# BrooksLabUCSC/splicedice

Measured on AMD Instinct MI355X. Metric: PS-matrix entries/sec (junctions x samples), higher is better.
Workload: dtype int32 counts -> f32 PS; 1 GPU; quant 2000000 junctions x 500 samples per GPU (north_star target size), cluster+PS; junctions_per_gpu=2000000, samples=500, counts=one seeded block of 200000 rows repeated down the matrix, parallelism=junction shards x1, one rank per GPU

## Files before the change

splicedice_amd/csrc/cluster_fast.hip:

```cpp
#include "common.h"

#ifndef SDICE_CLUSTER_ABLATE
#define SDICE_CLUSTER_ABLATE 0
#endif
#define SD_ABL(a, bit) (SDICE_CLUSTER_ABLATE && ((a).ablate & (bit)))

int sd_cluster_legacy(sdice_ctx* ctx, int64_t n, const int32_t* d_chrom, const int32_t* d_left, const int32_t* d_right,
                      const int8_t* d_strand, int32_t* d_row_of, int64_t* d_row_ptr, int64_t* nnz_out);

namespace {

constexpr int SPB = 8;
constexpr int BUCKET_MEAN = 2048;
constexpr int MAX_BUCKETS = 4096;
constexpr int SLOT_FACTOR = 8;
constexpr int64_t FAST_MAX_N = (int64_t)MAX_BUCKETS * BUCKET_MEAN;

enum : unsigned long long { ST_INVALID = 1, ST_SLOT_OVERFLOW = 2, ST_DUP = 4, ST_COL_OVERFLOW = 8, ST_LOOKBACK = 16 };
constexpr int SB_FLAGS = 0, SB_NNZ = 2, SB_MAXLEN = 32, SB_REACH = 64, SB_WORDS = 96;
constexpr int SB_STICKY = SB_WORDS, SB_ALLOC_WORDS = SB_WORDS + 8;
constexpr int SB_SLOTS = 32;

struct FastArgs {
    const int32_t* chrom; const int32_t* left; const int32_t* right; const int8_t* strand;
// ... 274 lines not shown
                for (int k = 0; k < K; ++k) {
                    const int kp = k ^ j;
                    if (kp > k) {
                        bool up;
                        if (k2 < K) up = (k & k2) == 0;
                        else if (k2 >= 64 * K) up = true;
                        else up = (lane & (k2 / K)) == 0;
                        const bool sw = up ? key[kp] < key[k] : key[kp] > key[k];
                        const uint64_t tk = key[k];
                        key[k] = sw ? key[kp] : tk;
                        key[kp] = sw ? tk : key[kp];
                    }
                }
            }
        }
    }
}

constexpr int SS_NB = 16;
constexpr int SS_MIN = 512, SS_MAX = 6400, SS_SUB_CAP = 1024;
constexpr int SS_KPT = (SS_MAX + SORT_T_ - 1) / SORT_T_;
static_assert((8192 - SS_MAX) * 8 >= SS_MAX * 2 && (8192 - SS_MAX) * 8 >= 256 * 12, "scratch behind the keys must hold the lists / the sample");

template <int K>
__device__ __forceinline__ void ss_sort_sub(const uint64_t* kb, const unsigned short* list, int n, int lane, uint64_t (&key)[16]) {
    uint64_t k_[K];
#pragma unroll
    for (int k = 0; k < K; ++k) {
        const int p = k * 64 + lane;
        k_[k] = p < n ? kb[list[p]] : ~0ull;
    }
    wave_sort_u64<K>(k_, lane);
#pragma unroll
    for (int k = 0; k < K; ++k) key[k] = k_[k];
}

__device__ __forceinline__ bool lds_sample_sort(uint64_t* kb, int count, int t) {
    __shared__ unsigned s_cnt[SS_NB], s_base[SS_NB + 1], s_max;
    __shared__ uint64_t s_spl[SS_NB];
    const int lane = t & 63, w = __builtin_amdgcn_readfirstlane(t >> 6);
    uint64_t* smp = kb + count;
    const int ns = count <= 2048 ? 128 : 256;
    const int per = ns / SS_NB;
    unsigned* rnk = reinterpret_cast<unsigned*>(smp + ns);
    unsigned short* list = reinterpret_cast<unsigned short*>(kb + count);
    __syncthreads();
    if (t < ns) { smp[t] = kb[(int)((int64_t)t * count / ns)]; rnk[t] = 0u; }
    if (t < SS_NB) s_cnt[t] = 0u;
    __syncthreads();
    {
        const int i = t & (ns - 1), chunk = SORT_T_ / ns, c = t / ns, len = ns / chunk;
        const uint64_t me = smp[i];
        unsigned below = 0;
        for (int j = c * len; j < c * len + len; ++j) below += smp[j] < me ? 1u : 0u;
        atomicAdd(&rnk[i], below);
    }
    __syncthreads();
    if (t < ns) {
        const unsigned r = rnk[t];
        if (r > 0 && r % (unsigned)per == 0) s_spl[r / (unsigned)per - 1] = smp[t];
    }
    __syncthreads();
    int where[SS_KPT];
#pragma unroll
    for (int q = 0; q < SS_KPT; ++q) {
        const int i = q * SORT_T_ + t;
        const bool act = i < count;
        int b = 0;
        if (act) {
            const uint64_t key = kb[i];
            int lo = 0, hi = SS_NB - 1;
            while (lo < hi) {
                const int mid = (lo + hi) >> 1;
                const bool le = s_spl[mid] <= key;
                lo = le ? mid + 1 : lo;
                hi = le ? hi : mid;
            }
            b = lo;
        }
        unsigned long long m = __ballot(act);
#pragma unroll
        for (int bit = 0; bit < 4; ++bit) {
            const unsigned long long bb = __ballot((b >> bit) & 1);
            m &= ((b >> bit) & 1) ? bb : ~bb;
        }
        unsigned basew = 0;
        if (act) {
            const int leader = __ffsll((long long)m) - 1;
            if (lane == leader) basew = atomicAdd(&s_cnt[b], (unsigned)__popcll(m));
            basew = (unsigned)__shfl((int)basew, leader);
        }
        where[q] = act ? (int)(((basew + (unsigned)__popcll(m & ((1ull << lane) - 1ull))) << 4) | (unsigned)b) : -1;
    }
    __syncthreads();
    if (w == 0) {
        const unsigned c = lane < SS_NB ? s_cnt[lane] : 0u;
        unsigned x = c, mx = c;
#pragma unroll
        for (int o = 1; o < SS_NB; o <<= 1) {
            const unsigned y = (unsigned)__shfl_up((int)x, o);
            if (lane >= o) x += y;
        }
#pragma unroll
        for (int o = 8; o > 0; o >>= 1) mx = max(mx, (unsigned)__shfl_xor((int)mx, o));
        if (lane < SS_NB) s_base[lane + 1] = x;
        if (lane == 0) { s_base[0] = 0u; s_max = mx; }
    }
    __syncthreads();
    if (s_max > (unsigned)SS_SUB_CAP) return false;
#pragma unroll
    for (int q = 0; q < SS_KPT; ++q)
        if (where[q] >= 0) list[s_base[where[q] & 15] + (unsigned)(where[q] >> 4)] = (unsigned short)(q * SORT_T_ + t);
    __syncthreads();
    const int n = (int)s_cnt[w];
    const unsigned base = s_base[w];
    uint64_t key[16];
    const int K = n <= 128 ? 2 : n <= 256 ? 4 : n <= 512 ? 8 : 16;
    if (K == 2) ss_sort_sub<2>(kb, list + base, n, lane, key);
    else if (K == 4) ss_sort_sub<4>(kb, list + base, n, lane, key);
    else if (K == 8) ss_sort_sub<8>(kb, list + base, n, lane, key);
    else ss_sort_sub<16>(kb, list + base, n, lane, key);
    __syncthreads();
#pragma unroll
    for (int k = 0; k < 16; ++k) {
        const int p = lane * K + k;
        if (k < K && p < n) kb[base + p] = key[k];
    }
    __syncthreads();
    return true;
}

constexpr int SORT_T = SORT_T_;
constexpr int SORT_WAVES = SORT_T / 64;
constexpr int RDX_CAP = 8192;
constexpr int RDX_IDX_BITS = 13;
constexpr int SORT_LDS_ELEMS = 4096;
constexpr size_t SORT_LDS_BYTES = (size_t)RDX_CAP * 8;
static_assert(SORT_LDS_BYTES >= (size_t)SORT_LDS_ELEMS * 16, "unpacked fallback must fit");

__device__ __forceinline__ int bits_u32(uint32_t v) { return v ? 32 - __clz(v) : 0; }

__global__ void __launch_bounds__(SORT_T, 8) bucket_sort_kernel(FastArgs a) {
    extern __shared__ uint4 lds_elems[];
    __shared__ unsigned long long wsum[SORT_WAVES];
    __shared__ uint32_t red[5][SORT_WAVES];
    __shared__ uint32_t s_dup;
    const int t = threadIdx.x, b = blockIdx.x, lane = t & 63, w = __builtin_amdgcn_readfirstlane(t >> 6);
    if (a.sb[SB_FLAGS] & (ST_INVALID | ST_SLOT_OVERFLOW)) return;
    const int count = (int)a.cursor[b];
    unsigned long long part = 0;
    for (int i = t; i < b; i += SORT_T) part += a.cursor[i];
#pragma unroll
    for (int o = 32; o > 0; o >>= 1) part += __shfl_xor(part, o);
    if (lane == 0) wsum[w] = part;
    if (t == 0) s_dup = 0;
    __syncthreads();
    int64_t start = 0;
    for (int k = 0; k < SORT_WAVES; ++k) start += (int64_t)wsum[k];
    if (count == 0) return;
    uint4* src = a.slots + (int64_t)b * a.slot_cap;

    int total_bits = 99, bl = 0, bn = 0;
    uint32_t cmin = 0, lmin = 0;
    const bool small = count <= RDX_CAP && count <= a.lds_cap;
    if (small) {
        uint32_t c0 = 0xffffffffu, c1 = 0, l0 = 0xffffffffu, l1 = 0, n1 = 0;
        for (int i = t; i < count; i += SORT_T) {
            const uint4 e = src[i];
            c0 = min(c0, e.x); c1 = max(c1, e.x); l0 = min(l0, e.y); l1 = max(l1, e.y); n1 = max(n1, (e.z >> 1) - e.y);
        }
#pragma unroll
        for (int o = 32; o > 0; o >>= 1) {
            c0 = min(c0, (uint32_t)__shfl_xor((int)c0, o)); c1 = max(c1, (uint32_t)__shfl_xor((int)c1, o));
            l0 = min(l0, (uint32_t)__shfl_xor((int)l0, o)); l1 = max(l1, (uint32_t)__shfl_xor((int)l1, o));
            n1 = max(n1, (uint32_t)__shfl_xor((int)n1, o));
        }
        if (lane == 0) { red[0][w] = c0; red[1][w] = c1; red[2][w] = l0; red[3][w] = l1; red[4][w] = n1; }
        __syncthreads();
        for (int k = 0; k < SORT_WAVES; ++k) {
            c0 = min(c0, red[0][k]); c1 = max(c1, red[1][k]); l0 = min(l0, red[2][k]); l1 = max(l1, red[3][k]);
            n1 = max(n1, red[4][k]);
        }
        cmin = c0; lmin = l0;
        bl = bits_u32(l1 - l0); bn = bits_u32(n1);
        total_bits = bits_u32(c1 - c0) + bl + bn + 1;
    }
    uint32_t dup = 0;
    auto emit_all = [&](auto get) {
        for (int i0 = 0; i0 < count; i0 += SORT_T) {
            const int i = i0 + t;
            const bool act = i < count;
            uint32_t rr = 0, blk = 0xffffffffu;
            if (act) {
                const uint4 e = get(i);
                const int64_t r = start + i;
                a.rowC[r] = e.x; a.rowL[r] = e.y; a.rowR2[r] = e.z;
                a.row_of[e.w] = (int32_t)r;
                rr = e.z >> 1;
                blk = (uint32_t)(r >> 6);
            }
            const uint32_t blk0 = (uint32_t)__shfl((int)blk, 0);
            uint32_t m0 = (act && blk == blk0) ? rr : 0u, m1 = (act && blk != blk0) ? rr : 0u;
#pragma unroll
            for (int o = 32; o > 0; o >>= 1) {
                m0 = max(m0, (uint32_t)__shfl_xor((int)m0, o));
                m1 = max(m1, (uint32_t)__shfl_xor((int)m1, o));
            }
            if (lane == 0 && blk0 != 0xffffffffu) {
                if (m0) atomicMax(&a.bmax64[blk0], m0);
                if (m1) atomicMax(&a.bmax64[blk0 + 1], m1);
            }
        }
    };
    if (small && total_bits + RDX_IDX_BITS <= 64) {
        uint64_t* kb0 = reinterpret_cast<uint64_t*>(lds_elems);
        for (int i = t; i < count; i += SORT_T) {
            const uint4 e = src[i];
            uint64_t k = (((uint64_t)(e.x - cmin) << bl) | (uint64_t)(e.y - lmin)) << bn;
            k = ((k | (uint64_t)((e.z >> 1) - e.y)) << 1) | (uint64_t)(e.z & 1u);
            kb0[i] = (k << RDX_IDX_BITS) | (uint64_t)i;
        }
        int P = 1;
        while (P < count) P <<= 1;
        bool sorted_already = false;
        if (a.sample_sort && count >= SS_MIN && count <= SS_MAX && !SD_ABL(a, 1)) sorted_already = lds_sample_sort(kb0, count, t);
        if (sorted_already) {}
        else if (P > 1 && !SD_ABL(a, 1)) bitonic_sort_u64(kb0, count, P, t, SORT_T); else __syncthreads();
        const uint64_t* sorted = kb0;
        for (int i = t; i + 1 < count; i += SORT_T)
            if ((sorted[i] >> RDX_IDX_BITS) == (sorted[i + 1] >> RDX_IDX_BITS)) dup = 1;
        if (!SD_ABL(a, 2)) emit_all([&](int i) { return src[sorted[i] & ((1u << RDX_IDX_BITS) - 1u)]; });
    } else {
        int P = 1;
        while (P < count) P <<= 1;
        uint4* buf;
        if (count <= SORT_LDS_ELEMS && count <= a.lds_cap) {
            for (int i = t; i < count; i += SORT_T) lds_elems[i] = src[i];
            buf = lds_elems;
            if (P > 1) bitonic_sort<true, uint4>(buf, count, P, t, SORT_T); else __syncthreads();
        } else {
            buf = src;
            bitonic_sort<false, uint4>(buf, count, P, t, SORT_T);
        }
        for (int i = t; i + 1 < count; i += SORT_T) {
            const uint4 e = buf[i], f = buf[i + 1];
            if (f.x == e.x && f.y == e.y && f.z == e.z) dup = 1;
        }
        emit_all([&](int i) { return buf[i]; });
    }
    if (dup) s_dup = 1;
    __syncthreads();
    if (t == 0 && s_dup) { atomicOr(&a.sb[SB_FLAGS], (unsigned long long)ST_DUP); atomicOr(&a.sb[SB_STICKY], (unsigned long long)ST_DUP); }
}

constexpr unsigned long long LB_A = 1ull << 62, LB_P = 2ull << 62, LB_MASK = (1ull << 62) - 1;

__device__ __forceinline__ unsigned long long ld_agent(const unsigned long long* p) {
    return __hip_atomic_load(p, __ATOMIC_RELAXED, __HIP_MEMORY_SCOPE_AGENT);
}
__device__ __forceinline__ void st_agent(unsigned long long* p, unsigned long long v) {
    __hip_atomic_store(p, v, __ATOMIC_RELAXED, __HIP_MEMORY_SCOPE_AGENT);
}

__device__ __forceinline__ unsigned long long lookback_exclusive(unsigned long long* state, int tile, unsigned long long agg,
                                                                 int lane, unsigned long long* sb, bool fail) {
    if (lane == 0) st_agent(&state[tile], (tile == 0 ? LB_P : LB_A) | agg);
    unsigned long long excl = 0;
    int idx = tile - 1;
    unsigned spins = fail && tile == 1 ? (1u << 21) : 0u;
    while (idx >= 0) {
        const int j = idx - lane;
        const unsigned long long v = j >= 0 ? ld_agent(&state[j]) : LB_P;
        const unsigned flag = (unsigned)(v >> 62);
        const unsigned long long empty = __ballot(flag == 0u);
        const unsigned long long pm = __ballot(flag == 2u);
        const int first_p = pm ? __ffsll((long long)pm) - 1 : 64;
        const unsigned long long need = first_p >= 63 ? ~0ull : ((1ull << (first_p + 1)) - 1ull);
        if ((empty & need) || (fail && tile == 1)) {
            if (++spins > (1u << 21)) {
                if (lane == 0) { atomicOr(&sb[SB_FLAGS], (unsigned long long)ST_LOOKBACK); atomicOr(&sb[SB_STICKY], (unsigned long long)ST_LOOKBACK); }
                break;
            }
            __builtin_amdgcn_s_sleep(2);
            continue;
        }
        unsigned long long x = lane <= first_p ? (v & LB_MASK) : 0ull;
#pragma unroll
        for (int o = 32; o > 0; o >>= 1) x += __shfl_xor(x, o);
        excl += x;
        if (first_p < 64) break;
        idx -= 64;
    }
    if (lane == 0 && tile != 0) st_agent(&state[tile], LB_P | (excl + agg));
    return excl;
}

template <int T>
struct NbCfg {
    static constexpr int HB = 256;
    static constexpr int HF = 128;
    static constexpr int W = T + HB + HF;
    static constexpr int STAGE = 11 * T;
    static constexpr int KMAX = 16;
    static constexpr int WIN_WORDS = 6 * W;
    static constexpr int UNION_WORDS = WIN_WORDS > STAGE ? WIN_WORDS : STAGE;
};

template <class Emit>
__device__ __forceinline__ void walk_back_global(const FastArgs& a, int q, uint32_t c, uint32_t l, uint32_t st, uint32_t maxlen,
                                                 Emit emit) {
    while (q >= 0) {
        const uint32_t qc = a.rowC[q], ql = a.rowL[q], qr = a.rowR2[q];
        if (qc != c || ql + maxlen < l) break;
        if ((q & 63) == 63 && a.bmax64[q >> 6] < l) { q -= 64; continue; }
        if ((qr & 1u) == st && (qr >> 1) >= l) emit(q);
        --q;
    }
}
template <class Emit>
__device__ __forceinline__ void walk_fwd_global(const FastArgs& a, int q, int n, uint32_t c, uint32_t rgt, uint32_t st, Emit emit) {
    while (q < n) {
        const uint32_t qc = a.rowC[q], ql = a.rowL[q], qr = a.rowR2[q];
        if (qc != c || ql > rgt) break;
        if ((qr & 1u) == st) emit(q);
        ++q;
    }
}

template <int T>
__global__ void __launch_bounds__(T, 8) neighbours_kernel(FastArgs a) {
    typedef NbCfg<T> Cfg;
    constexpr int W = Cfg::W, KMAX = Cfg::KMAX;
    constexpr int EPT = (W + T - 1) / T;
    __shared__ __align__(16) uint32_t u_mem[Cfg::UNION_WORDS];
    __shared__ int16_t tmp[(KMAX + 1) * T];
    __shared__ uint32_t wsum[T / 64];
    __shared__ unsigned long long wmax0[T / 64], wmax1[T / 64];
    __shared__ uint32_t s_misc[4];
    __shared__ unsigned long long s_base;
    unsigned long long* cL = reinterpret_cast<unsigned long long*>(u_mem);
    unsigned long long* pm = cL + W;
    uint32_t* wR = reinterpret_cast<uint32_t*>(pm + W);
    uint16_t* rid = reinterpret_cast<uint16_t*>(wR + W);
    uint16_t* pos = rid + W;
    int32_t* stage = reinterpret_cast<int32_t*>(u_mem);
    const int t = threadIdx.x, lane = t & 63, w = __builtin_amdgcn_readfirstlane(t >> 6);
    const int n = (int)a.n;
    const int n_tiles = (n + T - 1) / T;
    const bool failed_chain = (a.sb[SB_FLAGS] & (ST_INVALID | ST_SLOT_OVERFLOW | ST_DUP)) != 0;
    __shared__ int s_tile;
    unsigned long long* ticket = a.tile_state + n_tiles;
    if (t == 0) s_tile = failed_chain ? (int)blockIdx.x : (int)atomicAdd(ticket, 1ull);
    __syncthreads();
#pragma nounroll
    for (int tile = s_tile; tile < n_tiles;) {
    const int t0 = tile * T;
    const int nr = min(T, n - t0);
    if (failed_chain) {
        if (t < nr) { a.row_ptr[t0 + t] = 0; if ((t & 15) == 0) a.blkneed[(t0 + t) >> 4] = 0; }
        if (t0 + t == 0) a.row_ptr[n] = 0;
        tile += gridDim.x;
        continue;
    }
    if (t == 0) s_misc[2] = 0;
    if (t < 64) {
        unsigned long long m = t < SB_SLOTS ? a.sb[SB_MAXLEN + t] : 0ull;
#pragma unroll
        for (int o = 32; o > 0; o >>= 1) { const unsigned long long y = __shfl_xor(m, o); m = y > m ? y : m; }
        if (t == 0) s_misc[1] = (uint32_t)m;
    }
    const int wlo = max(0, t0 - Cfg::HB), whi = min(n, t0 + nr + Cfg::HF);
    const int wn = whi - wlo;
    const uint32_t c0w = a.rowC[wlo];
    const uint32_t l0w = a.rowL[wlo];
    const int64_t cap = a.col_cap;
    int n1 = 0;
    {
        unsigned long long comp[EPT], own_cl[EPT], r0 = 0, r1 = 0;
        uint32_t rr[EPT], str[EPT], c1 = 0;
        unsigned long long v0[EPT], v1[EPT];
        uint32_t cb[EPT];
#pragma unroll
        for (int e = 0; e < EPT; ++e) {
            const int i = t * EPT + e;
            comp[e] = 0; own_cl[e] = 0; rr[e] = 0; str[e] = 0;
            cb[e] = c1;
            if (i < wn) {
                const uint32_t rc = a.rowC[wlo + i] - c0w, r2 = a.rowR2[wlo + i];
                own_cl[e] = ((unsigned long long)rc << 32) | a.rowL[wlo + i];
                rr[e] = r2 >> 1; str[e] = r2 & 1u;
                comp[e] = ((unsigned long long)rc << 32) | rr[e];
                if (str[e]) { r1 = comp[e] > r1 ? comp[e] : r1; ++c1; } else { r0 = comp[e] > r0 ? comp[e] : r0; }
            }
            v0[e] = r0; v1[e] = r1;
        }
        unsigned long long x0 = r0, x1 = r1;
        uint32_t xc = c1;
#pragma unroll
        for (int o = 1; o < 64; o <<= 1) {
            const unsigned long long y0 = __shfl_up(x0, o), y1 = __shfl_up(x1, o);
            const uint32_t yc = __shfl_up(xc, o);
            if (lane >= o) { x0 = y0 > x0 ? y0 : x0; x1 = y1 > x1 ? y1 : x1; xc += yc; }
        }
        if (lane == 63) { wmax0[w] = x0; wmax1[w] = x1; wsum[w] = xc; }
        __syncthreads();
        unsigned long long p0 = __shfl_up(x0, 1), p1 = __shfl_up(x1, 1);
        uint32_t pc = xc - c1;
        if (lane == 0) { p0 = 0; p1 = 0; }
#pragma unroll
        for (int k = 0; k < T / 64; ++k) {
            if (k < w) { p0 = wmax0[k] > p0 ? wmax0[k] : p0; p1 = wmax1[k] > p1 ? wmax1[k] : p1; pc += wsum[k]; }
            n1 += (int)wsum[k];
        }
#pragma unroll
        for (int e = 0; e < EPT; ++e) {
            const int i = t * EPT + e;
            if (i < wn) {
                const int before1 = (int)(pc + cb[e]);
                const int k = str[e] ? W - 1 - before1 : i - before1;
                const unsigned long long m = str[e] ? (v1[e] > p1 ? v1[e] : p1) : (v0[e] > p0 ? v0[e] : p0);
                cL[k] = own_cl[e]; pm[k] = m; wR[k] = rr[e]; rid[k] = (uint16_t)i; pos[i] = (uint16_t)k;
            }
        }
    }
    __syncthreads();
    const uint32_t maxlen = s_misc[1];
    const int n0 = wn - n1;

    const int r = t0 + t;
    const int ri = r - wlo;
    const bool act = t < nr;
    int p = 0;
    unsigned long long own = 0;
    uint32_t rgt = 0;
    if (act) { p = pos[ri]; own = cL[p]; rgt = wR[p]; }
    const uint32_t st = p >= W - n1 ? 1u : 0u;
    const uint32_t l = (uint32_t)own, crel = (uint32_t)(own >> 32), c = crel + c0w;
    const unsigned long long tb = own;
    const unsigned long long tf = (own & 0xffffffff00000000ull) | rgt;
    const bool exact = wlo == 0 || crel != 0 || l0w + maxlen < l;
    const int dfw = st ? -1 : 1;
    const int first = st ? W - 1 : 0;
    const int last = st ? W - n1 : n0 - 1;

    uint32_t deg = 0;
    int far_b = r, far_f = r;
    bool redo = false;
    auto emit_far = [&](int q) {
        const int d = q - r;
        if (deg < (uint32_t)KMAX) {
            if (d >= -32768 && d <= 32767) tmp[deg * T + t] = (int16_t)d; else redo = true;
        }
        ++deg;
        if (d < 0) far_b = q; else far_f = q;
    };
    if (act && !SD_ABL(a, 64)) {
        int16_t* mytmp = tmp + t;
        auto take = [&](bool hit, int wi) {
            const uint32_t slot = (hit & (deg < (uint32_t)KMAX)) ? deg : (uint32_t)KMAX;
            mytmp[slot * T] = (int16_t)(wi - ri);
            deg += hit ? 1u : 0u;
            return hit ? wlo + wi : -1;
        };
        const int up = (p - first) * dfw, ulast = (last - first) * dfw;
        if (exact) {
            int u = up - 1;
            for (;;) {
                const int q0 = first + dfw * max(u, 0), q1 = first + dfw * max(u - 1, 0);
                const unsigned long long m0 = pm[q0], m1 = pm[q1];
                const uint32_t x0 = wR[q0], x1 = wR[q1];
                const int i0 = rid[q0], i1 = rid[q1];
                if (!((u >= 0) & (m0 >= tb))) break;
                const int f0 = take(x0 >= l, i0);
                far_b = f0 >= 0 ? f0 : far_b;
                --u;
                if (!((u >= 0) & (m1 >= tb))) break;
                const int f1 = take(x1 >= l, i1);
                far_b = f1 >= 0 ? f1 : far_b;
                --u;
            }
            if (u < 0 && wlo > 0) walk_back_global(a, wlo - 1, c, l, st, maxlen, emit_far);
        } else {
            walk_back_global(a, r - 1, c, l, st, maxlen, emit_far);
        }
        {
            int u = up + 1;
            for (;;) {
                const int q0 = first + dfw * min(u, ulast), q1 = first + dfw * min(u + 1, ulast);
                const unsigned long long c0 = cL[q0], c1 = cL[q1];
                const int i0 = rid[q0], i1 = rid[q1];
                if (!((u <= ulast) & (c0 <= tf))) break;
                far_f = take(true, i0);
                ++u;
                if (!((u <= ulast) & (c1 <= tf))) break;
                far_f = take(true, i1);
                ++u;
            }
            if (u > ulast && whi < n) walk_fwd_global(a, whi, n, c, rgt, st, emit_far);
        }
        if (deg > (uint32_t)KMAX) redo = true;
    }
    uint32_t reach = (uint32_t)max(r - far_b, far_f - r);
    {
        const int b16 = t & 15;
        const unsigned lo_n = act ? (unsigned)min(max(r - far_b - b16, 0), 255) : 0u;
        const unsigned hi_n = act ? (unsigned)min(max(far_f - r - (15 - b16), 0), 255) : 0u;
        typedef unsigned short us2 __attribute__((ext_vector_type(2)));
        us2 pk = {(unsigned short)lo_n, (unsigned short)hi_n};
#pragma unroll
        for (int o = 8; o > 0; o >>= 1) {
            const unsigned y = (unsigned)__shfl_xor((int)__builtin_bit_cast(unsigned, pk), o);
            pk = __builtin_elementwise_max(pk, __builtin_bit_cast(us2, y));
        }
        if (act && b16 == 0) a.blkneed[r >> 4] = (uint32_t)pk.x | ((uint32_t)pk.y << 8);
    }
    uint32_t x = deg;
#pragma unroll
    for (int o = 1; o < 64; o <<= 1) { const uint32_t y = __shfl_up(x, o); if (lane >= o) x += y; }
#pragma unroll
    for (int o = 32; o > 0; o >>= 1) reach = max(reach, (uint32_t)__shfl_xor((int)reach, o));
    if (lane == 63) wsum[w] = x;
    if (lane == 0 && reach) atomicMax(&s_misc[2], reach);
    __syncthreads();
    uint32_t wbase = 0, total = 0;
#pragma unroll
    for (int k = 0; k < T / 64; ++k) { const uint32_t v = wsum[k]; if (k < w) wbase += v; total += v; }
    const uint32_t loff = wbase + x - deg;
    if (w == 0) {
        const unsigned long long base = SD_ABL(a, 128) ? 0ull : lookback_exclusive(a.tile_state, tile, (unsigned long long)total, lane, a.sb, (a.ablate & 256) != 0);
        if (lane == 0) {
            s_base = base;
            if (s_misc[2]) atomicMax(&a.sb[SB_REACH + (tile % SB_SLOTS)], (unsigned long long)s_misc[2]);
        }
    }
    const bool staged = total <= (uint32_t)Cfg::STAGE;
    if (staged && act && deg) {
        if (!redo) {
            for (uint32_t k = 0; k < deg; ++k) stage[loff + k] = r + (int)tmp[k * T + t];
        } else {
            uint32_t k = loff;
            walk_back_global(a, r - 1, c, l, st, maxlen, [&](int q) { stage[k++] = q; });
            walk_fwd_global(a, r + 1, n, c, rgt, st, [&](int q) { stage[k++] = q; });
        }
    }
    __syncthreads();
    const int64_t base = (int64_t)s_base;
    if (act) a.row_ptr[r] = min(base + (int64_t)loff, cap);
    if (tile == n_tiles - 1 && t == 0) {
        a.row_ptr[n] = min(base + (int64_t)total, cap);
        a.sb[SB_NNZ] = (unsigned long long)(base + (int64_t)total);
        if (base + (int64_t)total > cap) { atomicOr(&a.sb[SB_FLAGS], (unsigned long long)ST_COL_OVERFLOW); atomicOr(&a.sb[SB_STICKY], (unsigned long long)ST_COL_OVERFLOW); }
    }
    if (staged) {
        for (uint32_t k = t; k < total; k += T)
            if (base + k < cap) a.col[base + k] = stage[k];
    } else if (act && deg) {
        int64_t k = base + loff;
        auto put = [&](int q) { if (k < cap) a.col[k] = q; ++k; };
        walk_back_global(a, r - 1, c, l, st, maxlen, put);
        walk_fwd_global(a, r + 1, n, c, rgt, st, put);
    }
    if (t == 0) s_tile = (int)atomicAdd(ticket, 1ull);
    __syncthreads();
    tile = s_tile;
    }
}

inline unsigned grid_for(int64_t n, int threads) { return (unsigned)sd_ceil_div(n, threads); }

struct FastPlan {
    FastArgs a;
    size_t zero_bytes;
    void* zero_base;
    size_t k4_zero_bytes;
    int n_tiles;
};

constexpr int NB_T = 512;

int fast_plan(sdice_ctx* ctx, int64_t n, const int32_t* d_chrom, const int32_t* d_left, const int32_t* d_right,
              const int8_t* d_strand, int32_t* d_row_of, int64_t* d_row_ptr, FastPlan& pl) {
    FastArgs& a = pl.a;
    a.chrom = d_chrom; a.left = d_left; a.right = d_right; a.strand = d_strand; a.n = n;
    static_assert(kSdParams[SD_P_CLUSTER_BUCKET_MEAN].dflt == BUCKET_MEAN, "the default is the largest mean the kernels take");
    int64_t bucket_mean = ctx->param(SD_P_CLUSTER_BUCKET_MEAN);
    if (bucket_mean < 256 || bucket_mean > BUCKET_MEAN) bucket_mean = BUCKET_MEAN;
    int64_t B = sd_ceil_div(n, bucket_mean);
    if (B < 1) B = 1;
    if (B > MAX_BUCKETS) B = MAX_BUCKETS;
    a.B = (int)B;
    a.spb = (int)ctx->param(SD_P_CLUSTER_SPB);
    if (a.spb < 2 || a.spb > 64) a.spb = n <= ((int64_t)2 << 20) ? 12 : SPB;
    a.S = B > 1 ? (int)(B * a.spb) : 0;
    const int64_t mean = sd_ceil_div(n, B);
    a.slot_cap = B > 1 ? (mean * SLOT_FACTOR < n ? mean * SLOT_FACTOR : n) : n;
    int64_t lds_cap = ctx->param(SD_P_CLUSTER_LDS_CAP);
    if (lds_cap <= 0 || lds_cap > 8192) lds_cap = 8192;
    if (lds_cap < 2) lds_cap = 2;
    a.lds_cap = (int)lds_cap;
    a.sample_sort = ctx->param(SD_P_CLUSTER_SAMPLE_SORT) != 0;
    pl.n_tiles = (int)sd_ceil_div(n, NB_T);
    const size_t nb64 = (size_t)sd_ceil_div(n, 64) + 2;
    if (!ctx->cluster_sb) {
        hipError_t e = hipMalloc((void**)&ctx->cluster_sb, (size_t)SB_ALLOC_WORDS * 8);
        if (e != hipSuccess) {
            sdice_set_error("sdice_cluster: hipMalloc of the status block failed: %s", hipGetErrorString(e));
            return SDICE_ERR_NOMEM;
        }
        SD_HIP(hipMemsetAsync(ctx->cluster_sb, 0, (size_t)SB_ALLOC_WORDS * 8, ctx->stream));
    }
    const size_t zk4 = ((size_t)pl.n_tiles + 2) * 8;
    const size_t n_cd = (size_t)(a.S + 255) / 256 + 4;
    const size_t zrest = (size_t)a.B * 4 + (size_t)(a.S + 4) * 4 + nb64 * 4 + n_cd * 4;
    const size_t slots_bytes = (size_t)a.B * (size_t)a.slot_cap * 16;
    const size_t total = zk4 + zrest + slots_bytes + (size_t)n * 12 + (size_t)a.B * 16 + 16 * 4096;
    SD_TRY(ctx->arena.reserve(total, ctx->stream));
    Arena& A = ctx->arena;
    char* z = (char*)A.alloc(zk4 + zrest + 1024);
    a.slots = (uint4*)A.alloc(slots_bytes);
    a.rowC = (uint32_t*)A.alloc((size_t)n * 4);
    a.rowL = (uint32_t*)A.alloc((size_t)n * 4);
    a.rowR2 = (uint32_t*)A.alloc((size_t)n * 4);
    a.spl = (uint64_t*)A.alloc((size_t)a.B * 8 + 8);
    if (!z || !a.slots || !a.rowC || !a.rowL || !a.rowR2 || !a.spl) return SDICE_ERR_NOMEM;
    pl.zero_base = z;
    pl.k4_zero_bytes = zk4;
    pl.zero_bytes = zk4 + zrest;
    a.sb = (unsigned long long*)ctx->cluster_sb;
    a.tile_state = (unsigned long long*)z;
    a.cursor = (uint32_t*)(z + zk4);
    a.rank = a.cursor + a.B;
    a.bmax64 = a.rank + a.S + 4;
    a.col_done = a.bmax64 + nb64;
    a.row_of = d_row_of; a.row_ptr = d_row_ptr;
    a.ablate = (int)ctx->param(SD_P_CLUSTER_ABLATE);
    return SDICE_OK;
}

int launch_neighbours(sdice_ctx* ctx, FastPlan& pl) {
    pl.a.col = ctx->d_col;
    pl.a.col_cap = ctx->col_cap;
    pl.a.blkneed = ctx->d_reach;
    static int per_cu = 0;
    if (per_cu == 0) {
        int occ = 0;
        SD_HIP(hipOccupancyMaxActiveBlocksPerMultiprocessor(&occ, reinterpret_cast<const void*>(neighbours_kernel<NB_T>), NB_T, 0));
        per_cu = occ > 0 ? occ : 1;
    }
    int64_t grid = std::min<int64_t>(pl.n_tiles, (int64_t)per_cu * ctx->n_cu);
    const int64_t forced = ctx->param(SD_P_CLUSTER_NB_GRID);
    if (forced > 0) grid = std::min<int64_t>(grid, forced);
    SD_LAUNCH(ctx, "neighbours_kernel", (neighbours_kernel<NB_T>), dim3((unsigned)std::max<int64_t>(grid, 1)), dim3(NB_T), 0, pl.a);
    return SDICE_OK;
}

int ensure_col(sdice_ctx* ctx, int64_t want) {
    if (want <= ctx->col_cap) return SDICE_OK;
    if (ctx->d_col) {
        SD_HIP(hipStreamSynchronize(ctx->stream));
        (void)hipFree(ctx->d_col);
    }
    ctx->d_col = nullptr;
    ctx->col_cap = 0;
    hipError_t e = hipMalloc((void**)&ctx->d_col, (size_t)want * 4);
    if (e != hipSuccess) {
        sdice_set_error("sdice_cluster: hipMalloc of %lld neighbour indices failed: %s", (long long)want, hipGetErrorString(e));
        return SDICE_ERR_NOMEM;
    }
    ctx->col_cap = want;
    return SDICE_OK;
}

int ensure_reach(sdice_ctx* ctx, int64_t n) {
    n = sd_ceil_div(n, 16) + 1;
    if (n <= ctx->reach_cap) return SDICE_OK;
    if (ctx->d_reach) {
        SD_HIP(hipStreamSynchronize(ctx->stream));
        (void)hipFree(ctx->d_reach);
    }
    ctx->d_reach = nullptr;
    ctx->reach_cap = 0;
    hipError_t e = hipMalloc((void**)&ctx->d_reach, (size_t)n * 4);
    if (e != hipSuccess) {
        sdice_set_error("sdice_cluster: hipMalloc of %lld block-reach entries failed: %s", (long long)n, hipGetErrorString(e));
        return SDICE_ERR_NOMEM;
    }
    ctx->reach_cap = n;
    return SDICE_OK;
}

}

static int fast_fetch_status(sdice_ctx* ctx, unsigned long long* flags, int64_t* nnz, int64_t* reach, unsigned long long* sticky = nullptr) {
    int64_t* hp = ctx->h_pinned;
    SD_HIP(hipMemcpyAsync(hp, ctx->cluster_sb, (size_t)SB_ALLOC_WORDS * 8, hipMemcpyDeviceToHost, ctx->stream));
    SD_HIP(hipMemsetAsync((unsigned long long*)ctx->cluster_sb + SB_STICKY, 0, 8, ctx->stream));
    SD_HIP(hipStreamSynchronize(ctx->stream));
    if (sticky) *sticky = (unsigned long long)hp[SB_STICKY];
    *flags = (unsigned long long)hp[SB_FLAGS];
    *nnz = hp[SB_NNZ];
    int64_t rc = 0;
    for (int i = 0; i < SB_SLOTS; ++i) rc = hp[SB_REACH + i] > rc ? hp[SB_REACH + i] : rc;
    *reach = rc;
    return SDICE_OK;
}

static int fast_flags_to_error(unsigned long long flags) {
    if (flags & ST_INVALID) {
        sdice_set_error("sdice_cluster: invalid junction (need 0 <= left <= right, chrom_rank >= 0, strand in {0,1})");
        return SDICE_ERR_ARG;
    }
    if (flags & ST_DUP) {
        sdice_set_error("sdice_cluster: duplicate junction (chrom, left, right, strand): the junctions must be distinct");
        return SDICE_ERR_ARG;
    }
    return SDICE_OK;
}

int sd_cluster_resolve(sdice_ctx* ctx) {
    if (!ctx->cluster_pending) return SDICE_OK;
    ctx->cluster_pending = false;
    unsigned long long flags = 0, sticky = 0;
    int64_t nnz = 0, reach = 0;
    SD_TRY(fast_fetch_status(ctx, &flags, &nnz, &reach, &sticky));
    ctx->nnz = 0;
    flags |= sticky;
    SD_TRY(fast_flags_to_error(flags));
    if (flags & (ST_SLOT_OVERFLOW | ST_LOOKBACK)) {
        sdice_set_error("sdice_cluster_dev (asynchronous): %s; call with nnz != NULL (synchronous) "
                        "to take the generic path", (flags & ST_LOOKBACK) ? "the look-back gave up waiting" : "a sort bucket overflowed");
        return SDICE_ERR_STATE;
    }
    if (flags & ST_COL_OVERFLOW) {
        sdice_set_error("sdice_cluster_dev (asynchronous): %lld neighbour entries exceed the list capacity %lld; "
                        "call once with nnz != NULL (synchronous) to size it", (long long)nnz, (long long)ctx->col_cap);
        return SDICE_ERR_STATE;
    }
    ctx->nnz = nnz;
    ctx->cluster_reach = (int)reach;
    return SDICE_OK;
}

extern "C" int sdice_cluster_status(sdice_ctx* ctx, int64_t* nnz, int32_t* reach) {
    SD_ARG(ctx, "ctx is NULL");
    SD_TRY(sd_cluster_resolve(ctx));
    if (nnz) *nnz = ctx->nnz;
    if (reach) *reach = ctx->cluster_reach;
    return SDICE_OK;
}

extern "C" int sdice_cluster_dev(sdice_ctx* ctx, int64_t n, const int32_t* d_chrom, const int32_t* d_left,
                                 const int32_t* d_right, const int8_t* d_strand, int32_t* d_row_of,
                                 int64_t* d_row_ptr, int64_t* nnz_out) {
    SD_ARG(ctx, "ctx is NULL");
    SD_ARG(n >= 0 && n < ((int64_t)1 << 31), "n out of range");
    SD_HIP(hipSetDevice(ctx->device));
    if (nnz_out && ctx->cluster_pending) SD_TRY(sd_cluster_resolve(ctx));
    ctx->reach_n = 0;
    const bool legacy = n > FAST_MAX_N || ctx->param(SD_P_CLUSTER_GENERIC) || ctx->param(SD_P_CLUSTER_LEGACY);
    if ((legacy || n == 0) && ctx->cluster_pending) SD_TRY(sd_cluster_resolve(ctx));
    if (legacy || n == 0) return sd_cluster_legacy(ctx, n, d_chrom, d_left, d_right, d_strand, d_row_of, d_row_ptr, nnz_out);
    SD_ARG(d_chrom && d_left && d_right && d_strand && d_row_of && d_row_ptr, "NULL pointer");
    ctx->nnz = 0;
    ctx->cluster_reach = 0;
    if (nnz_out) *nnz_out = 0;

    FastPlan pl;
    SD_TRY(fast_plan(ctx, n, d_chrom, d_left, d_right, d_strand, d_row_of, d_row_ptr, pl));
    FastArgs& a = pl.a;
    SD_TRY(ensure_col(ctx, 16 * n + 1024));
    SD_TRY(ensure_reach(ctx, n));

    SD_HIP(hipMemsetAsync(pl.zero_base, 0, pl.zero_bytes, ctx->stream));
    if (a.S == 0) SD_HIP(hipMemsetAsync(a.sb, 0, (size_t)SB_WORDS * 8, ctx->stream));
    if (a.S > 0) {
        const unsigned g = grid_for(a.S, 256);
        SD_LAUNCH(ctx, "sample_rank_kernel", sample_rank_kernel, dim3(g, g), dim3(256), 0, a);
    }
    {
        const size_t lds = (size_t)a.B * 16;
        if (n <= (1 << 19)) {
            SD_HIP(hipFuncSetAttribute(reinterpret_cast<const void*>(bucket_scatter_kernel<512>),
                                       hipFuncAttributeMaxDynamicSharedMemorySize, (int)lds));
            SD_LAUNCH(ctx, "bucket_scatter_kernel", (bucket_scatter_kernel<512>), dim3(grid_for(n, 512 * SC_KPT)), dim3(512), lds, a);
        } else {
            SD_HIP(hipFuncSetAttribute(reinterpret_cast<const void*>(bucket_scatter_kernel<1024>),
                                       hipFuncAttributeMaxDynamicSharedMemorySize, (int)lds));
            SD_LAUNCH(ctx, "bucket_scatter_kernel", (bucket_scatter_kernel<1024>), dim3(grid_for(n, 1024 * SC_KPT)), dim3(1024), lds, a);
        }
    }
    {
        const size_t lds = SORT_LDS_BYTES;
        SD_HIP(hipFuncSetAttribute(reinterpret_cast<const void*>(bucket_sort_kernel),
                                   hipFuncAttributeMaxDynamicSharedMemorySize, (int)lds));
        SD_LAUNCH(ctx, "bucket_sort_kernel", bucket_sort_kernel, dim3((unsigned)a.B), dim3(SORT_T), lds, a);
    }
    SD_TRY(launch_neighbours(ctx, pl));

    if (!nnz_out) {
        ctx->cluster_pending = true;
        ctx->reach_n = n;
        return SDICE_OK;
    }
    unsigned long long flags = 0;
    int64_t nnz = 0, reach = 0;
    SD_TRY(fast_fetch_status(ctx, &flags, &nnz, &reach));
    SD_TRY(fast_flags_to_error(flags));
    if (flags & (ST_SLOT_OVERFLOW | ST_LOOKBACK))
        return sd_cluster_legacy(ctx, n, d_chrom, d_left, d_right, d_strand, d_row_of, d_row_ptr, nnz_out);
    if (flags & ST_COL_OVERFLOW) {
        SD_TRY(sd_cluster_check_nnz(ctx, nnz, false));
        SD_TRY(ensure_col(ctx, nnz + nnz / 8 + 1024));
        SD_HIP(hipMemsetAsync(pl.zero_base, 0, pl.k4_zero_bytes, ctx->stream));
        SD_HIP(hipMemsetAsync(a.sb, 0, (size_t)SB_MAXLEN * 8, ctx->stream));
        SD_HIP(hipMemsetAsync(a.sb + SB_REACH, 0, (size_t)SB_SLOTS * 8, ctx->stream));
        SD_TRY(launch_neighbours(ctx, pl));
        SD_TRY(fast_fetch_status(ctx, &flags, &nnz, &reach));
        if (flags) {
            sdice_set_error("sdice_cluster: neighbour pass failed after resizing (flags %llu)", flags);
            return SDICE_ERR_STATE;
        }
    }
    ctx->nnz = nnz;
    ctx->cluster_reach = (int)reach;
    ctx->reach_n = n;
    *nnz_out = nnz;
    return SDICE_OK;
}
```

Before: 509.8 billion entries/s.

## Replace neighbour walks with binary-search forward extents and histogram-prefix backward counts

The neighbours kernel now binary-searches each window row's forward overlap extent in shared memory. Those extents feed a histogram and prefix sum, so each row knows up front how many backward neighbours it has. The backward walk stops once that count is reached, and forward neighbours come straight from the sorted window order, so the linear forward walk and the per-row prefix-max array are gone. The strand partition uses ballot/mbcnt instead of shuffle scans, and LDS use shrinks, which may raise occupancy. The cost is extra barriers, LDS atomics and binary-search steps per tile, plus more correctness risk around window edges.

```diff
diff --git a/splicedice_amd/csrc/cluster_fast.hip b/splicedice_amd/csrc/cluster_fast.hip
--- a/splicedice_amd/csrc/cluster_fast.hip
+++ b/splicedice_amd/csrc/cluster_fast.hip
@@ -600,7 +600,7 @@
     static constexpr int W = T + HB + HF;
     static constexpr int STAGE = 11 * T;
     static constexpr int KMAX = 16;
-    static constexpr int WIN_WORDS = 6 * W;
+    static constexpr int WIN_WORDS = 4 * W;
     static constexpr int UNION_WORDS = WIN_WORDS > STAGE ? WIN_WORDS : STAGE;
 };
 
@@ -630,17 +630,17 @@
     typedef NbCfg<T> Cfg;
     constexpr int W = Cfg::W, KMAX = Cfg::KMAX;
     constexpr int EPT = (W + T - 1) / T;
+    static_assert(EPT == 2, "the '-' counts of a wave's two sets of window rows are summed as one packed word");
     __shared__ __align__(16) uint32_t u_mem[Cfg::UNION_WORDS];
-    __shared__ int16_t tmp[(KMAX + 1) * T];
+    __shared__ int16_t tmp[KMAX * T];
+    __shared__ uint16_t rid[W];
     __shared__ uint32_t wsum[T / 64];
-    __shared__ unsigned long long wmax0[T / 64], wmax1[T / 64];
     __shared__ uint32_t s_misc[4];
     __shared__ unsigned long long s_base;
     unsigned long long* cL = reinterpret_cast<unsigned long long*>(u_mem);
-    unsigned long long* pm = cL + W;
-    uint32_t* wR = reinterpret_cast<uint32_t*>(pm + W);
-    uint16_t* rid = reinterpret_cast<uint16_t*>(wR + W);
-    uint16_t* pos = rid + W;
+    uint32_t* hs = reinterpret_cast<uint32_t*>(cL + W);
+    uint16_t* fu = reinterpret_cast<uint16_t*>(hs + W);
+    uint16_t* pos = fu + W;
     int32_t* stage = reinterpret_cast<int32_t*>(u_mem);
     const int t = threadIdx.x, lane = t & 63, w = __builtin_amdgcn_readfirstlane(t >> 6);
     const int n = (int)a.n;
@@ -649,6 +649,12 @@
     __shared__ int s_tile;
     unsigned long long* ticket = a.tile_state + n_tiles;
     if (t == 0) s_tile = failed_chain ? (int)blockIdx.x : (int)atomicAdd(ticket, 1ull);
+    if (t < 64) {
+        unsigned long long m = t < SB_SLOTS ? a.sb[SB_MAXLEN + t] : 0ull;
+#pragma unroll
+        for (int o = 32; o > 0; o >>= 1) { const unsigned long long y = __shfl_xor(m, o); m = y > m ? y : m; }
+        if (t == 0) s_misc[1] = (uint32_t)m;
+    }
     __syncthreads();
 #pragma nounroll
     for (int tile = s_tile; tile < n_tiles;) {
@@ -661,143 +667,147 @@
         continue;
     }
     if (t == 0) s_misc[2] = 0;
-    if (t < 64) {
-        unsigned long long m = t < SB_SLOTS ? a.sb[SB_MAXLEN + t] : 0ull;
-#pragma unroll
-        for (int o = 32; o > 0; o >>= 1) { const unsigned long long y = __shfl_xor(m, o); m = y > m ? y : m; }
-        if (t == 0) s_misc[1] = (uint32_t)m;
-    }
     const int wlo = max(0, t0 - Cfg::HB), whi = min(n, t0 + nr + Cfg::HF);
     const int wn = whi - wlo;
+    const int n_srch = t0 + nr - wlo;
     const uint32_t c0w = a.rowC[wlo];
     const uint32_t l0w = a.rowL[wlo];
     const int64_t cap = a.col_cap;
     int n1 = 0;
+    unsigned long long tfw[EPT];
+    uint32_t strw[EPT];
     {
-        unsigned long long comp[EPT], own_cl[EPT], r0 = 0, r1 = 0;
-        uint32_t rr[EPT], str[EPT], c1 = 0;
-        unsigned long long v0[EPT], v1[EPT];
-        uint32_t cb[EPT];
+        unsigned long long own_cl[EPT];
 #pragma unroll
         for (int e = 0; e < EPT; ++e) {
-            const int i = t * EPT + e;
-            comp[e] = 0; own_cl[e] = 0; rr[e] = 0; str[e] = 0;
-            cb[e] = c1;
+            const int i = t + e * T;
+            own_cl[e] = 0; tfw[e] = 0; strw[e] = 0;
             if (i < wn) {
                 const uint32_t rc = a.rowC[wlo + i] - c0w, r2 = a.rowR2[wlo + i];
                 own_cl[e] = ((unsigned long long)rc << 32) | a.rowL[wlo + i];
-                rr[e] = r2 >> 1; str[e] = r2 & 1u;
-                comp[e] = ((unsigned long long)rc << 32) | rr[e];
-                if (str[e]) { r1 = comp[e] > r1 ? comp[e] : r1; ++c1; } else { r0 = comp[e] > r0 ? comp[e] : r0; }
-            }
-            v0[e] = r0; v1[e] = r1;
-        }
-        unsigned long long x0 = r0, x1 = r1;
-        uint32_t xc = c1;
-#pragma unroll
-        for (int o = 1; o < 64; o <<= 1) {
-            const unsigned long long y0 = __shfl_up(x0, o), y1 = __shfl_up(x1, o);
-            const uint32_t yc = __shfl_up(xc, o);
-            if (lane >= o) { x0 = y0 > x0 ? y0 : x0; x1 = y1 > x1 ? y1 : x1; xc += yc; }
-        }
-        if (lane == 63) { wmax0[w] = x0; wmax1[w] = x1; wsum[w] = xc; }
+                tfw[e] = ((unsigned long long)rc << 32) | (r2 >> 1);
+                strw[e] = r2 & 1u;
+            }
+        }
+        const unsigned long long b0 = __ballot(strw[0] != 0u), b1 = __ballot(strw[1] != 0u);
+        uint32_t before[EPT];
+        before[0] = __builtin_amdgcn_mbcnt_hi((uint32_t)(b0 >> 32), __builtin_amdgcn_mbcnt_lo((uint32_t)b0, 0u));
+        before[1] = __builtin_amdgcn_mbcnt_hi((uint32_t)(b1 >> 32), __builtin_amdgcn_mbcnt_lo((uint32_t)b1, 0u));
+        if (lane == 0) wsum[w] = (uint32_t)__popcll(b0) | ((uint32_t)__popcll(b1) << 16);
+        for (int k = t; k < W; k += T) hs[k] = 0;
         __syncthreads();
-        unsigned long long p0 = __shfl_up(x0, 1), p1 = __shfl_up(x1, 1);
-        uint32_t pc = xc - c1;
-        if (lane == 0) { p0 = 0; p1 = 0; }
-#pragma unroll
-        for (int k = 0; k < T / 64; ++k) {
-            if (k < w) { p0 = wmax0[k] > p0 ? wmax0[k] : p0; p1 = wmax1[k] > p1 ? wmax1[k] : p1; pc += wsum[k]; }
-            n1 += (int)wsum[k];
-        }
+        uint32_t tot = 0, pre = 0;
+#pragma unroll
+        for (int k = 0; k < T / 64; ++k) { const uint32_t v = wsum[k]; if (k < w) pre += v; tot += v; }
+        const int tot0 = (int)(tot & 0xffffu);
+        n1 = tot0 + (int)(tot >> 16);
+        before[0] += pre & 0xffffu;
+        before[1] += (uint32_t)tot0 + (pre >> 16);
 #pragma unroll
         for (int e = 0; e < EPT; ++e) {
-            const int i = t * EPT + e;
+            const int i = t + e * T;
             if (i < wn) {
-                const int before1 = (int)(pc + cb[e]);
-                const int k = str[e] ? W - 1 - before1 : i - before1;
-                const unsigned long long m = str[e] ? (v1[e] > p1 ? v1[e] : p1) : (v0[e] > p0 ? v0[e] : p0);
-                cL[k] = own_cl[e]; pm[k] = m; wR[k] = rr[e]; rid[k] = (uint16_t)i; pos[i] = (uint16_t)k;
+                const int k = strw[e] ? W - 1 - (int)before[e] : i - (int)before[e];
+                cL[k] = own_cl[e]; rid[k] = (uint16_t)i; pos[i] = (uint16_t)k;
             }
         }
     }
     __syncthreads();
     const uint32_t maxlen = s_misc[1];
     const int n0 = wn - n1;
+
+    if (!SD_ABL(a, 64)) {
+        const int top = 1 << (31 - __clz(max(max(n0, n1), 1)));
+#pragma unroll
+        for (int e = 0; e < EPT; ++e) {
+            if (t + e * T < n_srch) {
+                const int ns = strw[e] ? n1 : n0;
+                const int sbase = strw[e] ? W : -1, sdir = strw[e] ? -1 : 1;
+                const unsigned long long tf = tfw[e];
+                int cnt = 0;
+#pragma nounroll
+                for (int step = top; step > 0; step >>= 1) {
+                    const int idx = cnt + step;
+                    const unsigned long long v = cL[sbase + sdir * min(idx, ns)];
+                    cnt = ((idx <= ns) & (v <= tf)) ? idx : cnt;
+                }
+                fu[pos[t + e * T]] = (uint16_t)(cnt - 1);
+                if (cnt < ns) atomicAdd(&hs[sbase + sdir * (cnt + 1)], 1u);
+            }
+        }
+        __syncthreads();
+        {
+            uint32_t h0 = 0, h1 = 0;
+            if (2 * t < W) { h0 = hs[2 * t]; h1 = hs[2 * t + 1]; }
+            uint32_t x = h0 + h1;
+#pragma unroll
+            for (int o = 1; o < 64; o <<= 1) { const uint32_t y = __shfl_up(x, o); if (lane >= o) x += y; }
+            if (lane == 63) wsum[w] = x;
+            __syncthreads();
+#pragma unroll
+            for (int k = 0; k < T / 64; ++k) { const uint32_t v = wsum[k]; if (k < w) x += v; }
+            if (2 * t < W) { hs[2 * t] = x - h1; hs[2 * t + 1] = x; }
+        }
+        __syncthreads();
+    }
 
     const int r = t0 + t;
     const int ri = r - wlo;
     const bool act = t < nr;
     int p = 0;
     unsigned long long own = 0;
-    uint32_t rgt = 0;
-    if (act) { p = pos[ri]; own = cL[p]; rgt = wR[p]; }
+    if (act) { p = pos[ri]; own = cL[p]; }
     const uint32_t st = p >= W - n1 ? 1u : 0u;
     const uint32_t l = (uint32_t)own, crel = (uint32_t)(own >> 32), c = crel + c0w;
-    const unsigned long long tb = own;
-    const unsigned long long tf = (own & 0xffffffff00000000ull) | rgt;
     const bool exact = wlo == 0 || crel != 0 || l0w + maxlen < l;
     const int dfw = st ? -1 : 1;
     const int first = st ? W - 1 : 0;
     const int last = st ? W - n1 : n0 - 1;
-
-    uint32_t deg = 0;
+    const int up = (p - first) * dfw;
+
+    uint32_t degb = 0, degf = 0;
     int far_b = r, far_f = r;
     bool redo = false;
-    auto emit_far = [&](int q) {
-        const int d = q - r;
-        if (deg < (uint32_t)KMAX) {
-            if (d >= -32768 && d <= 32767) tmp[deg * T + t] = (int16_t)d; else redo = true;
-        }
-        ++deg;
-        if (d < 0) far_b = q; else far_f = q;
-    };
     if (act && !SD_ABL(a, 64)) {
-        int16_t* mytmp = tmp + t;
-        auto take = [&](bool hit, int wi) {
-            const uint32_t slot = (hit & (deg < (uint32_t)KMAX)) ? deg : (uint32_t)KMAX;
-            mytmp[slot * T] = (int16_t)(wi - ri);
-            deg += hit ? 1u : 0u;
-            return hit ? wlo + wi : -1;
-        };
-        const int up = (p - first) * dfw, ulast = (last - first) * dfw;
         if (exact) {
+            const uint32_t below = st ? hs[W - 1] - (p > 0 ? hs[p - 1] : 0u) : hs[p];
+            const uint32_t want = (uint32_t)up - below;
+            int16_t* mytmp = tmp + t;
             int u = up - 1;
-            for (;;) {
-                const int q0 = first + dfw * max(u, 0), q1 = first + dfw * max(u - 1, 0);
-                const unsigned long long m0 = pm[q0], m1 = pm[q1];
-                const uint32_t x0 = wR[q0], x1 = wR[q1];
+            while ((degb < want) & (u >= 0)) {
+                const int q0 = first + dfw * u, q1 = first + dfw * max(u - 1, 0);
+                const int f0 = fu[q0], f1 = fu[q1];
                 const int i0 = rid[q0], i1 = rid[q1];
-                if (!((u >= 0) & (m0 >= tb))) break;
-                const int f0 = take(x0 >= l, i0);
-                far_b = f0 >= 0 ? f0 : far_b;
-                --u;
-                if (!((u >= 0) & (m1 >= tb))) break;
-                const int f1 = take(x1 >= l, i1);
-                far_b = f1 >= 0 ? f1 : far_b;
-                --u;
-            }
-            if (u < 0 && wlo > 0) walk_back_global(a, wlo - 1, c, l, st, maxlen, emit_far);
+                const bool hit0 = f0 >= up, hit1 = (u >= 1) & (f1 >= up);
+                if (hit0) mytmp[min(degb, (uint32_t)KMAX - 1u) * T] = (int16_t)(i0 - ri);
+                degb += hit0 ? 1u : 0u;
+                far_b = hit0 ? wlo + i0 : far_b;
+                if (hit1) mytmp[min(degb, (uint32_t)KMAX - 1u) * T] = (int16_t)(i1 - ri);
+                degb += hit1 ? 1u : 0u;
+                far_b = hit1 ? wlo + i1 : far_b;
+                u -= 2;
+            }
         } else {
-            walk_back_global(a, r - 1, c, l, st, maxlen, emit_far);
-        }
-        {
-            int u = up + 1;
-            for (;;) {
-                const int q0 = first + dfw * min(u, ulast), q1 = first + dfw * min(u + 1, ulast);
-                const unsigned long long c0 = cL[q0], c1 = cL[q1];
-                const int i0 = rid[q0], i1 = rid[q1];
-                if (!((u <= ulast) & (c0 <= tf))) break;
-                far_f = take(true, i0);
-                ++u;
-                if (!((u <= ulast) & (c1 <= tf))) break;
-                far_f = take(true, i1);
-                ++u;
-            }
-            if (u > ulast && whi < n) walk_fwd_global(a, whi, n, c, rgt, st, emit_far);
-        }
-        if (deg > (uint32_t)KMAX) redo = true;
-    }
+            walk_back_global(a, r - 1, c, l, st, maxlen, [&](int q) {
+                const int d = q - r;
+                if (degb < (uint32_t)KMAX) {
+                    if (d >= -32768) tmp[degb * T + t] = (int16_t)d; else redo = true;
+                }
+                ++degb;
+                far_b = q;
+            });
+        }
+        if (degb > (uint32_t)KMAX) redo = true;
+        const int f = fu[p];
+        degf = (uint32_t)(f - up);
+        if (degf) far_f = wlo + (int)rid[first + dfw * f];
+        if (f == (last - first) * dfw && whi < n) {
+            const uint32_t d0 = degf;
+            walk_fwd_global(a, whi, n, c, a.rowR2[r] >> 1, st, [&](int q) { ++degf; far_f = q; });
+            if (degf != d0) redo = true;
+        }
+    }
+    const uint32_t deg = degb + degf;
     uint32_t reach = (uint32_t)max(r - far_b, far_f - r);
     {
         const int b16 = t & 15;
@@ -834,11 +844,14 @@
     const bool staged = total <= (uint32_t)Cfg::STAGE;
     if (staged && act && deg) {
         if (!redo) {
-            for (uint32_t k = 0; k < deg; ++k) stage[loff + k] = r + (int)tmp[k * T + t];
+            for (uint32_t k = 0; k < degb; ++k) stage[loff + k] = r + (int)tmp[k * T + t];
+            int32_t* fwd = stage + loff + degb;
+            const uint16_t* nxt = rid + first + dfw * (up + 1);
+            for (uint32_t k = 0; k < degf; ++k) fwd[k] = wlo + (int)nxt[dfw * (int)k];
         } else {
             uint32_t k = loff;
             walk_back_global(a, r - 1, c, l, st, maxlen, [&](int q) { stage[k++] = q; });
-            walk_fwd_global(a, r + 1, n, c, rgt, st, [&](int q) { stage[k++] = q; });
+            walk_fwd_global(a, r + 1, n, c, a.rowR2[r] >> 1, st, [&](int q) { stage[k++] = q; });
         }
     }
     __syncthreads();
@@ -856,7 +869,7 @@
         int64_t k = base + loff;
         auto put = [&](int q) { if (k < cap) a.col[k] = q; ++k; };
         walk_back_global(a, r - 1, c, l, st, maxlen, put);
-        walk_fwd_global(a, r + 1, n, c, rgt, st, put);
+        walk_fwd_global(a, r + 1, n, c, a.rowR2[r] >> 1, st, put);
     }
     if (t == 0) s_tile = (int)atomicAdd(ticket, 1ull);
     __syncthreads();
```

Measured after the change: 520.1 billion entries/s, median of 6. 2.0% higher.
